# davidesantangelo/krep

Hardware: NVIDIA H100
Metric: GB/s scanned (HBM-resident corpus) (higher is better)
Workload: dtype u8

## Files before the change

krep_b200/csrc/engine.cu:

```cuda
#include <cub/device/device_radix_sort.cuh>
#include <algorithm>
#include <chrono>
#include <cstdarg>
#include <cstdio>
#include <cstdlib>
#include <cstring>
#include <mutex>
#include <thread>
#include "common.h"
#include "corpus.h"
#include "engine.h"

namespace kb {

static thread_local int t_err = 0;
static thread_local char t_errmsg[512] = "";

void set_error(int code, const char *fmt, ...)
{
    t_err = code;
    va_list ap;
    va_start(ap, fmt);
    vsnprintf(t_errmsg, sizeof t_errmsg, fmt, ap);
    va_end(ap);
// ... 128 lines not shown
    if (e != cudaSuccess)
    {
        cudaGetLastError();
        n = 0;
    }
    trace("cudaGetDeviceCount -> %d", n);
    g_visible = n > MAX_DEV ? MAX_DEV : n;
    return g_visible;
}

int primary_device()
{
    if (g_primary >= 0) return g_primary;
    if (visible_devices() == 0)
    {
        set_error(-1, "no CUDA device available; this engine has no CPU fallback");
        return -1;
    }
    int d = 0;
    if (cudaGetDevice(&d) != cudaSuccess) d = 0;
    g_primary = d;
    return d;
}

static int ctx_create(DevCtx &E, int device)
{
    trace("device %d: creating context", device);
    CK(cudaSetDevice(device));
    cudaDeviceProp prop;
    CK(cudaGetDeviceProperties(&prop, device));
    if (prop.major != 9 || prop.minor != 0)
    {
        set_error(-1, "device %d (%s, sm_%d%d) is not an sm_90 part; kernels are built for sm_90a only", device,
                  prop.name, prop.major, prop.minor);
        return -1;
    }
    E.device = device;
    E.sm_count = prop.multiProcessorCount;
    CK(cudaStreamCreateWithFlags(&E.scan_stream, cudaStreamNonBlocking));
    CK(cudaStreamCreateWithFlags(&E.copy_stream, cudaStreamNonBlocking));
    CK(cudaStreamCreateWithFlags(&E.fin_stream, cudaStreamNonBlocking));
    CK(cudaMalloc(&E.d_counter, 64 * SCAN_SLOTS));
    CK(cudaMemset(E.d_counter, 0, 64 * SCAN_SLOTS));
    CK(cudaEventCreate(&E.ev_ca));
    CK(cudaEventCreate(&E.ev_cb));
    for (int s = 0; s < SCAN_SLOTS; s++)
    {
        CK(cudaMalloc(&E.d_pack[s], (PACK_KEYS + 1) * sizeof(uint64_t)));
        CK(cudaHostAlloc(&E.h_pack[s], (PACK_KEYS + 1) * sizeof(uint64_t), cudaHostAllocMapped | cudaHostAllocPortable));
        E.h_pack[s][0] = 0;
        CK(cudaEventCreate(&E.ev_a[s]));
        CK(cudaEventCreate(&E.ev_b[s]));
        CK(cudaEventCreateWithFlags(&E.ev_done[s], cudaEventDisableTiming));
        CK(cudaEventCreateWithFlags(&E.ev_scanned[s], cudaEventDisableTiming));
        E.counter_clean[s] = true;
    }
    E.ready = true;
    trace("device %d: context ready (%s, %d SMs)", device, prop.name, E.sm_count);
    return 0;
}

DevCtx *ctx_get(int device)
{
    if (device < 0 || device >= MAX_DEV || device >= visible_devices())
    {
        set_error(-1, visible_devices() == 0 ? "no CUDA device available; this engine has no CPU fallback"
                                               : "CUDA device %d is not visible to this process",
                  device);
        return nullptr;
    }
    DevCtx &E = g_ctx[device];
    if (E.ready)
    {
        cudaSetDevice(device);
        return &E;
    }
    static std::mutex mu[MAX_DEV];
    std::lock_guard<std::mutex> lk(mu[device]);
    if (!E.ready && ctx_create(E, device) != 0) return nullptr;
    return &E;
}

DevCtx *ctx_primary()
{
    const int d = primary_device();
    return d < 0 ? nullptr : ctx_get(d);
}

static std::vector<Plan *> g_all_plans;
static std::mutex g_plans_mu;

static void ctx_destroy(DevCtx &E)
{
    if (!E.ready) return;
    cudaSetDevice(E.device);
    cudaDeviceSynchronize();
    for (int s = 0; s < SCAN_SLOTS; s++) cudaFree(E.d_list[s]);
    cudaFree(E.d_alt);
    cudaFree(E.d_sort_tmp);
    cudaFree(E.d_bounds);
    cudaFreeHost(E.h_bounds);
    cudaFreeHost(E.h_batch);
    cudaFree(E.d_rx_batch);
    cudaFree(E.d_counter);
    cudaFree(E.d_ring);
    cudaFree(E.d_line_recs);
    cudaFree(E.d_line_out);
    cudaFreeHost(E.h_line_out);
    cudaFreeHost(E.h_keys);
    regex_pack_free(E);
    for (int s = 0; s < SCAN_SLOTS; s++)
    {
        cudaFree(E.d_pack[s]);
        cudaFreeHost(E.h_pack[s]);
        cudaEventDestroy(E.ev_a[s]);
        cudaEventDestroy(E.ev_b[s]);
        cudaEventDestroy(E.ev_done[s]);
        cudaEventDestroy(E.ev_scanned[s]);
    }
    for (auto &s : E.stage) cudaFreeHost(s.buf);
    for (auto &s : E.stage)
        if (s.ev) cudaEventDestroy(s.ev);
    for (auto ev : E.ev_pool) cudaEventDestroy(ev);
    for (auto ev : E.ring_landed) cudaEventDestroy(ev);
    for (auto ev : E.ring_scanned) cudaEventDestroy(ev);
    cudaEventDestroy(E.ev_ca);
    cudaEventDestroy(E.ev_cb);
    cudaStreamDestroy(E.scan_stream);
    cudaStreamDestroy(E.copy_stream);
    cudaStreamDestroy(E.fin_stream);
    E = DevCtx();
}

void plan_cache_clear();

void engine_shutdown()
{
    std::lock_guard<std::recursive_mutex> lk(g_mu);
    DeviceGuard guard;
    plan_cache_clear();
    {
        std::lock_guard<std::mutex> lp(g_plans_mu);
        for (Plan *p : g_all_plans)
            for (int d = 0; d < MAX_DEV; d++)
            {
                PlanDev &pd = p->dev[d];
                if (!pd.ready) continue;
                cudaSetDevice(d);
                cudaFree(pd.d_pat_val);
                cudaFree(pd.d_pat_mask);
                if (pd.ac) ac_free_device(pd.ac);
                pd = PlanDev();
            }
    }
    for (int d = 0; d < MAX_DEV; d++) ctx_destroy(g_ctx[d]);
    g_primary = -1;
}

int ensure_keys(DevCtx &E, uint64_t cap)
{
    if (cap <= E.key_cap) return 0;
    uint64_t ncap = E.key_cap ? E.key_cap : (1ull << 20);
    while (ncap < cap) ncap *= 2;
    CK(cudaDeviceSynchronize());
    for (int s = 0; s < SCAN_SLOTS; s++)
    {
        cudaFree(E.d_list[s]);
        E.d_list[s] = nullptr;
    }
    cudaFree(E.d_alt);
// ... 350 lines not shown
int reset_counter(DevCtx &E, int slot, cudaStream_t stream)
{
    if (E.counter_clean[slot]) return 0;
    CK(cudaMemsetAsync(slot_counter(E, slot), 0, 64, stream));
    E.counter_clean[slot] = true;
    return 0;
}

static constexpr int FIN_THREADS = 512, FIN_SLICES = 16, FIN_KEYS = FIN_THREADS / FIN_SLICES, FIN_PIECE = 2048;

__global__ void __launch_bounds__(FIN_THREADS) k_finish(unsigned long long *counter, const uint64_t *__restrict__ keys, uint64_t cap,
                                                        uint64_t *d_pack, int want_sort)
{
    __shared__ uint64_t s_keys[FIN_PIECE];
    __shared__ unsigned long long s_cnt;
    if (threadIdx.x == 0) s_cnt = counter[0];
    __syncthreads();
    const unsigned long long cnt = s_cnt;
    if (blockIdx.x == 0 && threadIdx.x == 0) d_pack[0] = cnt;
    const bool sorting = want_sort && cnt != 0 && cnt <= PACK_KEYS && cnt <= cap;
    const uint32_t n = sorting ? (uint32_t)cnt : 0u;
    const uint32_t idx = blockIdx.x * FIN_KEYS + threadIdx.x / FIN_SLICES, slice = threadIdx.x % FIN_SLICES;
    if (blockIdx.x * FIN_KEYS < n)
    {
        const uint64_t mine = idx < n ? keys[idx] : ~0ull;
        uint32_t rank = 0;
        for (uint32_t base = 0; base < n; base += FIN_PIECE)
        {
            const uint32_t m = n - base < FIN_PIECE ? n - base : FIN_PIECE;
            for (uint32_t j = threadIdx.x; j < FIN_PIECE; j += FIN_THREADS) s_keys[j] = j < m ? keys[base + j] : ~0ull;
            __syncthreads();
            const uint32_t mr = (m + 63u) & ~63u;
#pragma unroll 8
            for (uint32_t j = slice; j < mr; j += FIN_SLICES) rank += s_keys[j] < mine ? 1u : 0u;
            __syncthreads();
        }
#pragma unroll
        for (int o = 1; o < FIN_SLICES; o <<= 1) rank += __shfl_xor_sync(0xffffffffu, rank, o);
        if (idx < n && slice == 0) d_pack[1 + rank] = mine;
    }
    __syncthreads();
    if (threadIdx.x == 0)
    {
        __threadfence();
        const unsigned long long done = atomicAdd(&counter[1], 1ULL);
        if (done == gridDim.x - 1)
        {
            counter[0] = 0;
            counter[1] = 0;
        }
    }
}

int finish_scan(DevCtx &E, int slot, int want_sort, cudaStream_t stream)
{
    k_finish<<<PACK_KEYS / FIN_KEYS, FIN_THREADS, 0, stream>>>(slot_counter(E, slot), E.d_list[slot], E.key_cap, E.d_pack[slot],
                                                                 (want_sort && E.d_list[slot]) ? 1 : 0);
    CK(cudaGetLastError());
    CK(cudaMemcpyAsync(E.h_pack[slot], E.d_pack[slot], (want_sort ? PACK_KEYS + 1 : 1) * sizeof(uint64_t), cudaMemcpyDeviceToHost, stream));
    CK(cudaEventRecord(E.ev_done[slot], stream));
    count_launch();
    E.counter_clean[slot] = true;
    return 0;
}

int sort_keys(DevCtx &E, int slot, uint64_t n, int end_bit, cudaStream_t stream, const uint64_t **sorted)
{
    *sorted = E.d_list[slot];
    if (n < 2) return 0;
    cub::DoubleBuffer<uint64_t> db(E.d_list[slot], E.d_alt);
    size_t need = 0;
    CK(cub::DeviceRadixSort::SortKeys(nullptr, need, db, (int64_t)n, 0, end_bit, stream));
    if (need > E.sort_tmp_bytes)
    {
        CK(cudaStreamSynchronize(stream));
        cudaFree(E.d_sort_tmp);
        E.d_sort_tmp = nullptr;
        E.sort_tmp_bytes = 0;
        CK(cudaMalloc(&E.d_sort_tmp, need));
        E.sort_tmp_bytes = need;
    }
    CK(cub::DeviceRadixSort::SortKeys(E.d_sort_tmp, need, db, (int64_t)n, 0, end_bit, stream));
    *sorted = db.Current();
    return 0;
}

static int bits_for(uint64_t v)
{
    int b = 1;
    while (b < 64 && (v >> b)) b++;
    return b;
}

int key_end_bit(const Plan *plan, uint64_t max_offset, bool regex_matches)
{
    const int shift = plan->is_ac ? AC_END_SHIFT : regex_matches ? REGEX_MATCH_SHIFT : LIT_TAG_BITS;
    int b = bits_for(max_offset) + shift;
    return b > 64 ? 64 : b;
}

__global__ void __launch_bounds__(256) k_line_bounds(const uint8_t *__restrict__ text, uint64_t avail, uint64_t go,
                                                     const uint64_t *__restrict__ keys, uint64_t n, int is_ac, int has_prev,
                                                     int has_next, uint64_t *__restrict__ out)
{
    const uint64_t i = ((uint64_t)blockIdx.x * blockDim.x + threadIdx.x) >> 5;
    const int lane = threadIdx.x & 31;
    if (i >= n) return;
    auto start_of = [&](uint64_t key) -> uint64_t {
        if (!is_ac) return (key >> LIT_TAG_BITS) - go;
        return (key >> AC_END_SHIFT) - (1024 - ((key >> AC_LEN_SHIFT) & 1023)) - go;
    };
    const uint64_t s = start_of(keys[i]);
    const uint64_t lb = (!is_ac && i > 0) ? start_of(keys[i - 1]) : 0;
// ... 34 lines not shown
            break;
        }
    }
    if (lane == 0)
    {
        out[2 * i] = ls;
        out[2 * i + 1] = le;
    }
}

static int line_bounds(DevCtx &E, const Plan *plan, const krep_b200_shard_t *sh, const uint64_t *d_sorted, uint64_t n,
                       cudaStream_t stream, const uint64_t **d_bounds)
{
    *d_bounds = nullptr;
    if (n == 0) return 0;
    if (2 * n > E.bounds_cap)
    {
        CK(cudaStreamSynchronize(stream));
        cudaFree(E.d_bounds);
        E.d_bounds = nullptr;
        E.bounds_cap = 0;
        const uint64_t cap = 2 * n + n / 4 + 1024;
        CK(cudaMalloc(&E.d_bounds, cap * sizeof(uint64_t)));
        E.bounds_cap = cap;
    }
    const uint64_t threads = n * 32;
    const int has_prev = sh->prev_byte >= 0 && sh->prev_byte != '\n';
    const int has_next = sh->next_byte >= 0 && sh->next_byte != '\n';
    k_line_bounds<<<(unsigned)((threads + 255) / 256), 256, 0, stream>>>((const uint8_t *)sh->d_text, sh->avail_len, sh->global_offset,
                                                                        d_sorted, n, plan->is_ac ? 1 : 0, has_prev, has_next, E.d_bounds);
    CK(cudaGetLastError());
    count_launch();
    *d_bounds = E.d_bounds;
    return 0;
}

int scan_begin(DevCtx &E, const Plan *plan, const krep_b200_shard_t *sh, int want_positions, cudaStream_t stream, int *slot_out)
{
    if (!stream) stream = E.scan_stream;
    if (want_positions && ensure_keys(E, 1) != 0) return -2;
    const int slot = E.next_slot;
    if (E.pend[slot].active)
    {
        set_error(-3, "krep_b200_scan_shard_begin: %d scans are already in flight on device %d", SCAN_SLOTS, E.device);
        return -3;
    }
    CK(cudaStreamWaitEvent(stream, E.ev_done[slot], 0));
    if (reset_counter(E, slot, stream) != 0) return -2;
    CK(cudaEventRecord(E.ev_a[slot], stream));
    int rc = launch_scan(E, plan, sh, want_positions, stream, slot);
    if (rc != 0) return rc;
    CK(cudaEventRecord(E.ev_b[slot], stream));
    CK(cudaGetLastError());
    if (finish_scan(E, slot, want_positions, stream) != 0) return -2;
    PendingScan &P = E.pend[slot];
    P.active = true;
    P.plan = plan;
    P.shard = *sh;
    P.want_positions = want_positions;
    P.stream = stream;
    E.next_slot = (slot + 1) % SCAN_SLOTS;
    *slot_out = slot;
    return 0;
}

int scan_end(DevCtx &E, int slot, ScanOut *out)
{
    PendingScan &P = E.pend[slot];
    if (slot < 0 || slot >= SCAN_SLOTS || !P.active)
    {
        set_error(-3, "krep_b200_scan_shard_end: no scan in flight in slot %d", slot);
        return -3;
    }
    P.active = false;
    const Plan *plan = P.plan;
    const krep_b200_shard_t *sh = &P.shard;
    cudaStream_t stream = P.stream;
    reset_kernel_ms();
    for (int attempt = 0; attempt < 3; attempt++)
    {
        CK(cudaEventSynchronize(E.ev_done[slot]));
        const uint64_t cnt = E.h_pack[slot][0];
        float ms = 0.f;
        cudaEventElapsedTime(&ms, E.ev_a[slot], E.ev_b[slot]);
        add_kernel_ms(ms);
        *out = ScanOut();
        out->count = cnt;
        out->device = E.device;
        out->serial = ++E.serial;
        E.result_stream = stream;
        if (!P.want_positions) return 0;
        if (cnt <= E.key_cap)
        {
            int rc = 0;
            out->stored = cnt;
            if (cnt <= PACK_KEYS)
            {
                out->d_keys = E.d_pack[slot] + 1;
                out->h_sorted = E.h_pack[slot] + 1;
            }
            else
                rc = sort_keys(E, slot, cnt, key_end_bit(plan, sh->global_offset + sh->avail_len), stream, &out->d_keys);
            if (rc == 0 && plan->count_lines) rc = line_bounds(E, plan, sh, out->d_keys, cnt, stream, &out->d_bounds);
            return rc;
        }
        out->overflow = 1;
        for (int s2 = 0; s2 < SCAN_SLOTS; s2++)
            if (s2 != slot && E.pend[s2].active)
            {
                set_error(-3, "krep_b200_scan_shard_end: the occurrence list overflowed while another scan is in flight; end each "
                              "scan before beginning the next until the list has grown");
                return -3;
            }
        if (ensure_keys(E, cnt + cnt / 8 + 1024) != 0) return -2;
        if (reset_counter(E, slot, stream) != 0) return -2;
        CK(cudaEventRecord(E.ev_a[slot], stream));
        int rc = launch_scan(E, plan, sh, 1, stream, slot);
        if (rc != 0) return rc;
        CK(cudaEventRecord(E.ev_b[slot], stream));
        if (finish_scan(E, slot, 1, stream) != 0) return -2;
    }
    set_error(-4, "occurrence list kept overflowing");
    return -4;
}

int scan_shard(DevCtx &E, const Plan *plan, const krep_b200_shard_t *sh, int want_positions, cudaStream_t stream, ScanOut *out)
{
    int slot = 0;
    int rc = scan_begin(E, plan, sh, want_positions, stream, &slot);
    if (rc != 0) return rc;
    return scan_end(E, slot, out);
}

int fetch_keys(DevCtx &E, const ScanOut &so, const uint64_t **h)
{
    *h = nullptr;
    if (so.stored == 0) return 0;
    if (so.h_sorted)
    {
        *h = so.h_sorted;
        return 0;
    }
    if (so.stored > E.h_keys_cap)
    {
        cudaFreeHost(E.h_keys);
        E.h_keys = nullptr;
        E.h_keys_cap = 0;
        uint64_t cap = so.stored + so.stored / 4;
        if (cap < (1u << 16)) cap = 1u << 16;
        CK(cudaMallocHost(&E.h_keys, cap * sizeof(uint64_t)));
        E.h_keys_cap = cap;
    }
    cudaStream_t s = E.result_stream ? E.result_stream : E.scan_stream;
    CK(cudaMemcpyAsync(E.h_keys, so.d_keys, so.stored * sizeof(uint64_t), cudaMemcpyDeviceToHost, s));
    CK(cudaStreamSynchronize(s));
    *h = E.h_keys;
    return 0;
}

uint64_t merge_key_lists(const uint64_t *const *lists, const uint64_t *counts, uint32_t n_lists, uint64_t *dst)
{
    uint64_t total = 0;
    std::vector<uint64_t> cut;
    for (uint32_t i = 0; i < n_lists; i++)
    {
        if (counts[i] == 0) continue;
        if (dst + total != lists[i]) memmove(dst + total, lists[i], counts[i] * sizeof(uint64_t));
        cut.push_back(total);
        total += counts[i];
    }
    for (size_t i = 1; i < cut.size(); i++)
        if (dst[cut[i] - 1] > dst[cut[i]]) std::inplace_merge(dst, dst + cut[i], dst + (i + 1 < cut.size() ? cut[i + 1] : total));
    return total;
// ... 384 lines not shown
```

krep_b200/csrc/engine.h:

```cpp
#pragma once
#include <mutex>
#include <vector>
#include "common.h"

namespace kb {

static constexpr uint32_t PACK_KEYS = 16384;
static constexpr int SCAN_SLOTS = 2;

struct StageSlot
{
    uint8_t *buf = nullptr;
    cudaEvent_t ev = nullptr;
    bool in_flight = false;
};

struct PendingScan
{
    bool active = false;
    const Plan *plan = nullptr;
    krep_b200_shard_t shard;
    int want_positions = 0;
    cudaStream_t stream = nullptr;
};

struct RegexPackBufs;

struct DevCtx
{
    bool ready = false;
    int device = 0, sm_count = 0;
    cudaStream_t scan_stream = nullptr, copy_stream = nullptr;
    cudaStream_t fin_stream = nullptr;
    unsigned long long *d_counter = nullptr;
    bool counter_clean[SCAN_SLOTS] = {false, false};
    uint64_t *d_list[SCAN_SLOTS] = {nullptr, nullptr};
    uint64_t *d_alt = nullptr;
    uint64_t key_cap = 0;
    void *d_sort_tmp = nullptr;
    size_t sort_tmp_bytes = 0;
    uint64_t *d_bounds = nullptr;
    uint64_t bounds_cap = 0;
    uint64_t *h_bounds = nullptr;
    uint64_t h_bounds_cap = 0;
    uint64_t *d_pack[SCAN_SLOTS] = {nullptr, nullptr}, *h_pack[SCAN_SLOTS] = {nullptr, nullptr};
    cudaEvent_t ev_a[SCAN_SLOTS] = {nullptr, nullptr}, ev_b[SCAN_SLOTS] = {nullptr, nullptr};
    cudaEvent_t ev_done[SCAN_SLOTS] = {nullptr, nullptr};
    cudaEvent_t ev_scanned[SCAN_SLOTS] = {nullptr, nullptr};
    cudaEvent_t ev_ca = nullptr, ev_cb = nullptr;
    PendingScan pend[SCAN_SLOTS];
    int next_slot = 0;
    uint64_t serial = 0;
    cudaStream_t result_stream = nullptr;
    void *d_line_recs = nullptr;
    uint64_t line_recs_cap = 0;
    uint64_t *d_line_out = nullptr, *h_line_out = nullptr;
    uint64_t line_out_cap = 0;
    uint8_t *d_ring = nullptr;
    size_t ring_slot_bytes = 0;
    int ring_slots = 0;
    std::vector<cudaEvent_t> ring_landed, ring_scanned;
    std::vector<StageSlot> stage;
    size_t stage_bytes = 0;
    std::vector<cudaEvent_t> ev_pool;
    uint64_t *h_keys = nullptr;
    uint64_t h_keys_cap = 0;
    uint8_t *h_batch = nullptr;
    uint64_t h_batch_cap = 0;
    uint8_t *d_rx_batch = nullptr;
    size_t rx_batch_cap = 0;
    RegexPackBufs *rx_pack = nullptr;
};

struct RegexPackStats
{
    float scan_ms = 0.f, pack_ms = 0.f;
    uint64_t packed_bytes = 0;
};
int regex_scan_keys(DevCtx &E, const Plan *plan, const krep_b200_shard_t *shard, int mode, const char *who, uint64_t *cnt,
                    const uint64_t **d_sorted, uint64_t *device_lines);
int regex_pack_row(DevCtx &E, const krep_b200_shard_t *sh, int mode, const uint64_t *d_keys, uint64_t nkeys,
                   uint64_t device_lines, const void **d_row, uint64_t *row_bytes, float *pack_ms);
uint8_t *regex_pack_host_buffer(DevCtx &E, uint64_t bytes);
void regex_pack_free(DevCtx &E);

struct ErrState
{
    int code = 0;
    char msg[512] = "";
};
void get_error(ErrState *e);
void adopt_error(const ErrState &e);

std::recursive_mutex &engine_mutex();
int primary_device();
int visible_devices();
DevCtx *ctx_get(int device);
DevCtx *ctx_primary();
void engine_shutdown();
void prewarm_host_path(DevCtx &C);
void keep_devices_visible();
void warm_join();
bool warm_running();

struct DeviceGuard
{
    int saved = -1;
    DeviceGuard() { if (cudaGetDevice(&saved) != cudaSuccess) { saved = -1; cudaGetLastError(); } }
    ~DeviceGuard() { if (saved >= 0) cudaSetDevice(saved); }
};

Plan *plan_build(const search_params_t *P, int algo, bool only_matching);
Plan *regex_plan_build(const search_params_t *P, std::string *why);
void plan_free(Plan *p);
const PlanDev *plan_on_device(const Plan *p, DevCtx &C);
int resolve_algo(const search_params_t *P, int algo);

unsigned long long *slot_counter(DevCtx &C, int slot);
int scan_begin(DevCtx &C, const Plan *plan, const krep_b200_shard_t *sh, int want_positions, cudaStream_t stream, int *slot);
int scan_end(DevCtx &C, int slot, ScanOut *out);
int scan_shard(DevCtx &C, const Plan *plan, const krep_b200_shard_t *sh, int want_positions, cudaStream_t stream, ScanOut *out);
int finish_scan(DevCtx &C, int slot, int want_sort, cudaStream_t stream);
int ensure_keys(DevCtx &C, uint64_t cap);
int reset_counter(DevCtx &C, int slot, cudaStream_t stream);
int sort_keys(DevCtx &C, int slot, uint64_t n, int end_bit, cudaStream_t stream, const uint64_t **sorted);
int key_end_bit(const Plan *plan, uint64_t max_offset, bool regex_matches = false);
int fetch_keys(DevCtx &C, const ScanOut &so, const uint64_t **h);
void add_kernel_ms(float ms);
void reset_kernel_ms();
float get_kernel_ms();
void set_kernel_ms(float ms);
void trace(const char *fmt, ...);

bool count_lines_eligible(const Plan *plan, const search_params_t *P, int algo);
int ensure_line_out(DevCtx &C, uint64_t n);
int launch_count_lines(DevCtx &C, const Plan *plan, const krep_b200_shard_t *sh, cudaStream_t stream, uint64_t index);
uint64_t combine_line_records(const uint64_t *recs, size_t n);

uint64_t merge_key_lists(const uint64_t *const *lists, const uint64_t *counts, uint32_t n_lists, uint64_t *dst);

}
```

krep_b200/csrc/scan_count.cu:

```cuda
#include <algorithm>
#include "engine.h"
#include "lit_filters.cuh"

namespace kb {

enum : uint32_t
{
    LR_HAS_HIT = 1,
    LR_FIRST_OPEN = 2,
    LR_LAST_PENDING = 4,
    LR_HAS_NL = 8
};

struct LineRec
{
    uint32_t lines, flags;
};

struct CountDev
{
    LitDevParams p;
    uint64_t own_end;
    uint32_t part_groups, n_parts;
    uint32_t exact;
    uint32_t tail;
    LineRec *recs;
};

struct PartState
{
    uint32_t lines = 0;
    bool has_hit = false, first_open = false, pending = false, seen_nl = false;
    uint64_t covered_to = 0;
};

__device__ __noinline__ unsigned verify_exact_call(const LitDevParams &p, long long cand) { return verify_exact(p, cand); }

__device__ __forceinline__ uint32_t nl_nibble(uint32_t w)
{
    const uint32_t x = w ^ 0x0A0A0A0Au;
    const uint32_t y = ~(((x & 0x7F7F7F7Fu) + 0x7F7F7F7Fu) | x | 0x7F7F7F7Fu);
    return ((y >> 7) * 0x10204080u) >> 28;
}
__device__ __forceinline__ uint32_t nl_mask16(const uint4 &v)
{
    return nl_nibble(v.x) | (nl_nibble(v.y) << 4) | (nl_nibble(v.z) << 8) | (nl_nibble(v.w) << 12);
}
__device__ __forceinline__ uint32_t range_mask16(uint64_t unit, uint64_t lo, uint64_t hi)
{
    uint32_t m = 0xFFFFu;
    if (unit < lo) m = lo - unit >= 16 ? 0u : (m & ~((1u << (uint32_t)(lo - unit)) - 1u));
    if (unit + 16 > hi) m = hi <= unit ? 0u : (m & ((1u << (uint32_t)(hi - unit)) - 1u));
    return m;
}

__device__ __noinline__ bool scan_for_newline(const LitDevParams &p, uint64_t lo, uint64_t hi)
{
    const uint32_t lane = threadIdx.x & 31;
    if (hi > p.avail_len) hi = p.avail_len;
    for (uint64_t base = lo & ~15ull; base < hi; base += 512)
    {
        const uint64_t unit = base + 16ull * lane;
        uint32_t nm = 0;
        if (unit < hi && unit + 16 > lo)
        {
            if (unit + 16 <= p.avail_len) nm = nl_mask16(__ldg(reinterpret_cast<const uint4 *>(p.text + unit)));
            else
                for (uint64_t q = unit; q < p.avail_len; q++) nm |= (p.text[q] == '\n' ? 1u : 0u) << (uint32_t)(q - unit);
            nm &= range_mask16(unit, lo, hi);
        }
        if (__any_sync(0xffffffffu, nm != 0)) return true;
    }
    return false;
}

__device__ __forceinline__ void settle(const LitDevParams &p, PartState &S, uint64_t upto)
{
    if (S.covered_to < upto && (S.pending || (!S.has_hit && !S.seen_nl)))
        if (scan_for_newline(p, S.covered_to, upto))
        {
            S.pending = false;
            S.seen_nl = true;
        }
}

__device__ __forceinline__ void account(PartState &S, uint32_t hm, uint32_t nm)
{
    const uint32_t lane = threadIdx.x & 31;
    const bool has_nl = nm != 0;
    const uint32_t fnl = has_nl ? (uint32_t)__ffs(nm) - 1 : 0, lnl = has_nl ? 31u - (uint32_t)__clz(nm) : 0;
    const bool f = has_nl && (hm & ((1u << fnl) - 1u)) != 0;
    const bool l = has_nl && ((hm >> lnl) >> 1) != 0;
    uint32_t inner = 0;
    if (__popc(nm) >= 2)
    {
        uint32_t prev = fnl, rest = nm & (nm - 1);
        while (rest)
        {
            const uint32_t nx = (uint32_t)__ffs(rest) - 1;
            if (hm & (((1u << nx) - 1u) & ~((2u << prev) - 1u))) inner++;
            prev = nx;
            rest &= rest - 1;
        }
    }
    const uint32_t A = __ballot_sync(0xffffffffu, has_nl), T = __ballot_sync(0xffffffffu, !has_nl && hm != 0);
    const uint32_t F = __ballot_sync(0xffffffffu, f), Lm = __ballot_sync(0xffffffffu, l);
    uint32_t innersum = 0;
    if (__ballot_sync(0xffffffffu, inner != 0)) innersum = __reduce_add_sync(0xffffffffu, inner);
    if (A == 0)
    {
        if (T)
        {
            if (!S.pending)
            {
                S.lines++;
                if (!S.has_hit && !S.seen_nl) S.first_open = true;
            }
            S.pending = true;
            S.has_hit = true;
        }
        return;
    }
    const uint32_t j1 = (uint32_t)__ffs(A) - 1, jr = 31u - (uint32_t)__clz(A);
    if ((T & ((1u << j1) - 1u)) || ((F >> j1) & 1u))
    {
        if (!S.pending)
        {
            S.lines++;
            if (!S.has_hit && !S.seen_nl) S.first_open = true;
        }
        S.has_hit = true;
    }
    S.pending = false;
    S.seen_nl = true;
    bool gap = false;
    if (has_nl && lane != j1)
    {
        const uint32_t below = A & ((1u << lane) - 1u);
        const uint32_t pj = 31u - (uint32_t)__clz(below);
        const uint32_t between = ((1u << lane) - 1u) & ~((2u << pj) - 1u);
        gap = ((Lm >> pj) & 1u) || (T & between) || f;
    }
    const uint32_t G = __ballot_sync(0xffffffffu, gap);
    S.lines += (uint32_t)__popc(G) + innersum;
    if (G || innersum) S.has_hit = true;
    if (((Lm >> jr) & 1u) || ((T >> jr) >> 1))
    {
        S.lines++;
        S.has_hit = true;
        S.pending = true;
    }
}

__device__ __forceinline__ uint64_t pack_state(const PartState &S)
{
    return (uint64_t)S.lines | ((uint64_t)((S.has_hit ? 1u : 0u) | (S.first_open ? 2u : 0u) | (S.pending ? 4u : 0u) | (S.seen_nl ? 8u : 0u)) << 32);
}
__device__ __forceinline__ void unpack_state(uint64_t k, PartState &S)
{
    S.lines = (uint32_t)k;
    const uint32_t f = (uint32_t)(k >> 32);
    S.has_hit = f & 1u;
    S.first_open = f & 2u;
    S.pending = f & 4u;
    S.seen_nl = f & 8u;
}
__device__ __noinline__ uint64_t account_call(uint64_t packed, uint32_t hm, uint32_t nm)
{
    PartState S;
    unpack_state(packed, S);
    account(S, hm, nm);
    return pack_state(S);
}

template <bool WINDOW>
__device__ __noinline__ uint32_t hit_mask16(const CountDev &D, uint64_t unit, const uint4 &v, uint32_t nx)
{
    const LitDevParams &p = D.p;
    const uint32_t w[5] = {v.x, v.y, v.z, v.w, nx};
    uint32_t hm = 0;
    if (WINDOW)
    {
        const uint32_t mask = p.fold & p.win_mask, k0 = p.K[0];
#pragma unroll
        for (int k = 0; k < 4; k++)
#pragma unroll
            for (int r = 0; r < 4; r++)
            {
                const uint32_t win = r == 0 ? w[k] : __funnelshift_r(w[k], w[k + 1], 8 * r);
                if ((win & mask) == k0)
                {
                    const uint64_t st = unit + 4 * k + r;
                    const bool ok = D.exact ? (st >= p.own_begin && st < p.own_end && st + p.m <= p.avail_len)
                                            : verify_exact_call(p, (long long)st) != 0;
                    if (ok) hm |= 1u << (4 * k + r);
                }
            }
    }
    else
    {
#pragma unroll
        for (int k = 0; k < 4; k++)
#pragma unroll
            for (int d = 0; d < 4; d++)
                if ((w[k] & p.fold) == p.K[d] && verify_exact_call(p, (long long)(unit + 4 * k) - d)) hm |= 1u << (4 * k);
    }
    return hm;
}

__device__ __noinline__ PartState count_tail(const CountDev &D, PartState S, uint64_t cov, uint64_t nl_lo, uint64_t nl_hi, bool window)
{
    const LitDevParams &p = D.p;
    const uint32_t lane = threadIdx.x & 31;
    if (p.avail_len < p.emit_len && cov >= nl_hi) return S;
    const uint64_t last_start = p.avail_len >= p.emit_len ? p.avail_len - p.emit_len : 0;
    uint64_t end = nl_hi > last_start + 1 ? nl_hi : last_start + 1;
    if (!window && end < cov + 1) end = cov + 1;
    for (uint64_t base = cov; base < end; base += 32)
    {
        settle(p, S, base > nl_lo ? base : nl_lo);
        const uint64_t q = base + lane;
        uint32_t hm = 0, nm = 0;
        if (q < end)
        {
            if (p.avail_len >= p.emit_len && q >= p.tail_start && q <= last_start && verify_exact(p, (long long)q)) hm = 1;
            if (!window && q == cov && p.avail_len >= p.emit_len)
                for (uint64_t s = p.tail_start; s < cov && s <= last_start; s++)
                    if (verify_exact(p, (long long)s)) hm = 1;
            if (q >= nl_lo && q < nl_hi && q < p.avail_len && p.text[q] == '\n') nm = 1;
            if (nm) hm = 0;
        }
        account(S, hm, nm);
        S.covered_to = base + 32;
    }
    return S;
}

#ifndef KREP_B200_COUNT_MINB
#define KREP_B200_COUNT_MINB 3
#endif
template <bool WINDOW, bool FOLD, bool MASKED>
__global__ void __launch_bounds__(256, KREP_B200_COUNT_MINB) k_count_lines(const __grid_constant__ CountDev D)
{
    const LitDevParams &p = D.p;
    const uint4 *__restrict__ t4 = reinterpret_cast<const uint4 *>(p.text);
    const uint32_t lane = threadIdx.x & 31;
    const uint32_t warp_global = (blockIdx.x * blockDim.x + threadIdx.x) >> 5, total_warps = (gridDim.x * blockDim.x) >> 5;
    const uint32_t k0 = p.K[0], k1 = p.K[1], k2 = p.K[2], k3 = p.K[3], fold = p.fold, mask = p.win_mask;
    const uint32_t c1 = p.mulc[0], c2 = p.mulc[1], c3 = p.mulc[2];
    for (uint32_t pi = warp_global; pi < D.n_parts; pi += total_warps)
    {
        const uint64_t ga = p.group_begin + (uint64_t)pi * D.part_groups;
        uint64_t gb = ga + D.part_groups;
        if (gb > p.group_end) gb = p.group_end;
        const bool last_part = pi + 1 == D.n_parts;
        const uint64_t nl_lo = ga * 16 > p.own_begin ? ga * 16 : p.own_begin;
        const uint64_t nl_hi = (last_part || gb * 16 > D.own_end) ? D.own_end : gb * 16;
        PartState S;
        S.covered_to = nl_lo;
        for (uint64_t g = ga; g < gb; g += 128)
        {
            uint4 v[4];
            uint32_t nx[4];
            bool ok[4];
#pragma unroll
            for (int u = 0; u < 4; u++)
            {
                const uint64_t gi = g + 32 * u + lane;
                ok[u] = gi < gb;
                v[u] = ok[u] ? ld_stream(t4 + gi) : make_uint4(0u, 0u, 0u, 0u);
                nx[u] = 0;
                if (WINDOW && ok[u] && (lane == 31 || gi + 1 >= gb)) nx[u] = __ldg(reinterpret_cast<const uint32_t *>(t4 + gi + 1));
            }
            uint32_t cand = 0;
#pragma unroll
            for (int u = 0; u < 4; u++)
            {
                bool h;
                if (WINDOW)
                {
                    const uint32_t nb = __shfl_down_sync(0xffffffffu, v[u].x, 1);
                    if (!(lane == 31 || g + 32 * u + lane + 1 >= gb)) nx[u] = nb;
                    h = hit_vec_w<FOLD, MASKED>(v[u], nx[u], fold, mask, k0, c1, c2, c3);
                }
                else
                    h = hit_vec<FOLD>(v[u], fold, k0, k1, k2, k3);
                cand |= (h && ok[u]) ? (1u << u) : 0u;
            }
            const uint32_t any = __reduce_or_sync(0xffffffffu, cand);
            if (any)
            {
                const uint64_t tile_lo = g * 16;
                settle(p, S, tile_lo > nl_lo ? tile_lo : nl_lo);
                const bool inside = tile_lo >= nl_lo && tile_lo + 2048 <= nl_hi;
                uint64_t st = pack_state(S);
#pragma unroll
                for (int u = 0; u < 4; u++)
                {
                    const uint64_t unit = tile_lo + 512ull * u + 16ull * lane;
                    uint32_t hm = 0, nm = 0;
                    if (ok[u])
                    {
                        if ((cand >> u) & 1u) hm = hit_mask16<WINDOW>(D, unit, v[u], nx[u]);
                        nm = nl_mask16(v[u]);
                        if (!inside) nm &= range_mask16(unit, nl_lo, nl_hi);
                    }
                    st = account_call(st, hm, nm);
                }
                unpack_state(st, S);
                S.covered_to = tile_lo + 2048;
            }
        }
        if (last_part && D.tail) S = count_tail(D, S, gb * 16, nl_lo, nl_hi, WINDOW);
        uint32_t flags = 0;
        if (S.has_hit)
        {
            if (S.pending && S.covered_to < nl_hi && scan_for_newline(p, S.covered_to, nl_hi)) S.pending = false;
            flags = LR_HAS_HIT | (S.first_open ? LR_FIRST_OPEN : 0u) | (S.pending ? LR_LAST_PENDING : 0u) | LR_HAS_NL;
        }
        else
        {
            const bool nl = S.seen_nl || (S.covered_to < nl_hi && scan_for_newline(p, S.covered_to, nl_hi));
            flags = nl ? LR_HAS_NL : 0u;
        }
        if (lane == 0) D.recs[pi] = LineRec{S.lines, flags};
    }
}

__host__ __device__ __forceinline__ void append_rec(uint64_t &lines, uint32_t &flags, uint64_t blines, uint32_t bflags)
{
    const bool ah = flags & LR_HAS_HIT, bh = bflags & LR_HAS_HIT;
    if (!bh)
    {
        if (ah && (bflags & LR_HAS_NL)) flags &= ~(uint32_t)LR_LAST_PENDING;
        flags |= bflags & LR_HAS_NL;
        return;
    }
    if (!ah)
    {
        const bool had_nl = flags & LR_HAS_NL;
        lines = blines;
        flags = bflags | LR_HAS_NL * had_nl;
        if (had_nl) flags &= ~(uint32_t)LR_FIRST_OPEN;
        return;
    }
    lines += blines;
    if ((flags & LR_LAST_PENDING) && (bflags & LR_FIRST_OPEN)) lines--;
    flags = LR_HAS_HIT | LR_HAS_NL | (flags & LR_FIRST_OPEN) | (bflags & LR_LAST_PENDING);
}

__global__ void __launch_bounds__(1024) k_count_finish(const LineRec *recs, uint32_t n, uint64_t *d_out, uint64_t *h_out)
{
    __shared__ uint64_t s_lines[1024];
    __shared__ uint32_t s_flags[1024];
    const uint32_t per = (n + blockDim.x - 1) / blockDim.x;
    const uint32_t a = threadIdx.x * per, b = a + per < n ? a + per : n;
    uint64_t lines = 0;
    uint32_t flags = 0;
    for (uint32_t i = a; i < b; i++) append_rec(lines, flags, recs[i].lines, recs[i].flags);
    s_lines[threadIdx.x] = lines;
    s_flags[threadIdx.x] = flags;
    __syncthreads();
    if (threadIdx.x == 0)
    {
        lines = 0;
        flags = 0;
        for (uint32_t t = 0; t < blockDim.x; t++) append_rec(lines, flags, s_lines[t], s_flags[t]);
        d_out[0] = lines;
        d_out[1] = flags;
        h_out[0] = lines;
        h_out[1] = flags;
    }
}

#define CKC(call)                                                                                  \
    do                                                                                             \
    {                                                                                              \
        cudaError_t e_ = (call);                                                                   \
// ... 37 lines not shown
        set_error(-3, "shard text pointer must be 16-byte aligned");
        return -3;
    }
    const PlanDev *pd = plan_on_device(plan, E);
    if (!pd) return -2;
    if (ensure_line_out(E, index + 1) != 0) return -2;
    CountDev D;
    memset(&D, 0, sizeof D);
    LitDevParams &p = D.p;
    const uint64_t own_end = sh->own_end < sh->avail_len ? sh->own_end : sh->avail_len;
    p.text = (const uint8_t *)sh->d_text;
    p.avail_len = sh->avail_len;
    p.own_begin = sh->own_begin;
    p.own_end = own_end;
    p.global_offset = sh->global_offset;
    p.prev_byte = sh->prev_byte;
    p.next_byte = sh->next_byte;
    uint64_t total_groups;
    const bool window = plan->filter == FILTER_WINDOW4;
    if (!window)
    {
        total_groups = sh->avail_len / 16;
        p.tail_start = total_groups ? total_groups * 16 - 3 : 0;
    }
    else
    {
        total_groups = sh->avail_len >= 20 ? (sh->avail_len - 20) / 16 + 1 : 0;
        p.tail_start = total_groups * 16;
    }
    p.group_begin = sh->own_begin / 16;
    p.group_end = (own_end + 2) / 16 + 1;
    D.tail = p.group_end > total_groups ? 1u : 0u;
    if (p.group_end > total_groups) p.group_end = total_groups;
    if (p.group_begin > p.group_end) p.group_begin = p.group_end;
    p.m = plan->m;
    p.emit_len = plan->emit_len;
    for (int d = 0; d < 4; d++) p.K[d] = plan->K[d];
    p.fold = plan->fold;
    p.win_mask = plan->win_mask;
    p.mulc[0] = 1u << 24;
    p.mulc[1] = 1u << 16;
    p.mulc[2] = 1u << 8;
    p.pat_val = pd->d_pat_val;
    p.pat_mask = pd->d_pat_mask;
    p.whole_word = plan->whole_word;
    D.own_end = own_end;
    {
        bool letters = true;
        for (unsigned char ch : plan->pattern) letters &= is_alpha_c(ch);
        D.exact = (window && plan->m <= 4 && plan->whole_word == 0 && (plan->case_sensitive || letters)) ? 1u : 0u;
    }
    const uint64_t groups = p.group_end - p.group_begin;
    const char *v = getenv("KREP_B200_COUNT_PART_KB");
    const uint32_t kb_ = v && atoi(v) > 0 ? (uint32_t)atoi(v) : 64;
    uint64_t part = std::max<uint32_t>(128, kb_ * 64 / 128 * 128);
    const uint64_t max_parts = 1u << 18;
    if ((groups + part - 1) / part > max_parts) part = ((groups + max_parts - 1) / max_parts + 127) / 128 * 128;
    D.part_groups = (uint32_t)part;
    D.n_parts = (uint32_t)std::max<uint64_t>((groups + part - 1) / part, 1);
    if (D.n_parts > E.line_recs_cap)
    {
        CKC(cudaStreamSynchronize(stream));
        cudaFree(E.d_line_recs);
        E.d_line_recs = nullptr;
        E.line_recs_cap = 0;
        const uint64_t cap = std::max<uint64_t>(D.n_parts, 1u << 16);
        CKC(cudaMalloc(&E.d_line_recs, cap * sizeof(LineRec)));
        E.line_recs_cap = cap;
    }
    D.recs = (LineRec *)E.d_line_recs;
    const bool folded = plan->fold != 0xFFFFFFFFu, masked = plan->win_mask != 0xFFFFFFFFu;
    const uint64_t want_blocks = ((uint64_t)D.n_parts + 7) / 8;
    const unsigned grid = (unsigned)std::min<uint64_t>(want_blocks, (uint64_t)E.sm_count * KREP_B200_COUNT_MINB);
    if (!window)
    {
        if (folded) k_count_lines<false, true, false><<<grid, 256, 0, stream>>>(D);
        else k_count_lines<false, false, false><<<grid, 256, 0, stream>>>(D);
    }
    else if (folded)
    {
        if (masked) k_count_lines<true, true, true><<<grid, 256, 0, stream>>>(D);
        else k_count_lines<true, true, false><<<grid, 256, 0, stream>>>(D);
    }
    else
    {
        if (masked) k_count_lines<true, false, true><<<grid, 256, 0, stream>>>(D);
        else k_count_lines<true, false, false><<<grid, 256, 0, stream>>>(D);
    }
    CKC(cudaGetLastError());
    k_count_finish<<<1, 1024, 0, stream>>>(D.recs, D.n_parts, E.d_line_out + 2 * index, E.h_line_out + 2 * index);
    CKC(cudaGetLastError());
    count_launch(2);
    return 0;
}

uint64_t combine_line_records(const uint64_t *recs, size_t n)
{
    uint64_t lines = 0;
    uint32_t flags = 0;
    for (size_t i = 0; i < n; i++) append_rec(lines, flags, recs[2 * i], (uint32_t)recs[2 * i + 1]);
    return lines;
}

}
```

Baseline: 3108.

## Rewrite line-count accounting with per-lane bit tricks and async readback stream

Replaces the warp-wide PartState accounting (many ballots, noinline calls, settle scans) with a per-lane LaneCount using a carry-propagation bit trick to count hit lines, deferring first-line/newline resolution to the end of each partition. The hit-mask construction is templated on fold/mask and made branch-free, with verification only on candidate bits. Separately, the pack readback copy is moved to a dedicated finish stream, and the default count partition size grows from 64 KB to 256 KB. It risks correctness subtleties in the new line-boundary logic and reduced parallelism from larger partitions.

```diff
diff --git a/krep_b200/csrc/engine.cu b/krep_b200/csrc/engine.cu
--- a/krep_b200/csrc/engine.cu
+++ b/krep_b200/csrc/engine.cu
@@ -204,6 +204,7 @@
         CK(cudaEventCreate(&E.ev_a[s]));
         CK(cudaEventCreate(&E.ev_b[s]));
         CK(cudaEventCreateWithFlags(&E.ev_done[s], cudaEventDisableTiming));
+        CK(cudaEventCreateWithFlags(&E.ev_fin[s], cudaEventDisableTiming));
         CK(cudaEventCreateWithFlags(&E.ev_scanned[s], cudaEventDisableTiming));
         E.counter_clean[s] = true;
     }
@@ -268,6 +269,7 @@
         cudaEventDestroy(E.ev_a[s]);
         cudaEventDestroy(E.ev_b[s]);
         cudaEventDestroy(E.ev_done[s]);
+        cudaEventDestroy(E.ev_fin[s]);
         cudaEventDestroy(E.ev_scanned[s]);
     }
     for (auto &s : E.stage) cudaFreeHost(s.buf);
@@ -724,13 +726,20 @@
     }
 }
 
-int finish_scan(DevCtx &E, int slot, int want_sort, cudaStream_t stream)
+int finish_scan(DevCtx &E, int slot, int want_sort, cudaStream_t stream, cudaStream_t readback)
 {
     k_finish<<<PACK_KEYS / FIN_KEYS, FIN_THREADS, 0, stream>>>(slot_counter(E, slot), E.d_list[slot], E.key_cap, E.d_pack[slot],
                                                                  (want_sort && E.d_list[slot]) ? 1 : 0);
     CK(cudaGetLastError());
-    CK(cudaMemcpyAsync(E.h_pack[slot], E.d_pack[slot], (want_sort ? PACK_KEYS + 1 : 1) * sizeof(uint64_t), cudaMemcpyDeviceToHost, stream));
-    CK(cudaEventRecord(E.ev_done[slot], stream));
+    cudaStream_t cs = stream;
+    if (readback)
+    {
+        CK(cudaEventRecord(E.ev_fin[slot], stream));
+        CK(cudaStreamWaitEvent(readback, E.ev_fin[slot], 0));
+        cs = readback;
+    }
+    CK(cudaMemcpyAsync(E.h_pack[slot], E.d_pack[slot], (want_sort ? PACK_KEYS + 1 : 1) * sizeof(uint64_t), cudaMemcpyDeviceToHost, cs));
+    CK(cudaEventRecord(E.ev_done[slot], cs));
     count_launch();
     E.counter_clean[slot] = true;
     return 0;
@@ -871,7 +880,7 @@
     if (rc != 0) return rc;
     CK(cudaEventRecord(E.ev_b[slot], stream));
     CK(cudaGetLastError());
-    if (finish_scan(E, slot, want_positions, stream) != 0) return -2;
+    if (finish_scan(E, slot, want_positions, stream, E.fin_stream) != 0) return -2;
     PendingScan &P = E.pend[slot];
     P.active = true;
     P.plan = plan;
@@ -937,7 +946,7 @@
         int rc = launch_scan(E, plan, sh, 1, stream, slot);
         if (rc != 0) return rc;
         CK(cudaEventRecord(E.ev_b[slot], stream));
-        if (finish_scan(E, slot, 1, stream) != 0) return -2;
+        if (finish_scan(E, slot, 1, stream, E.fin_stream) != 0) return -2;
     }
     set_error(-4, "occurrence list kept overflowing");
     return -4;
diff --git a/krep_b200/csrc/engine.h b/krep_b200/csrc/engine.h
--- a/krep_b200/csrc/engine.h
+++ b/krep_b200/csrc/engine.h
@@ -46,6 +46,7 @@
     uint64_t *d_pack[SCAN_SLOTS] = {nullptr, nullptr}, *h_pack[SCAN_SLOTS] = {nullptr, nullptr};
     cudaEvent_t ev_a[SCAN_SLOTS] = {nullptr, nullptr}, ev_b[SCAN_SLOTS] = {nullptr, nullptr};
     cudaEvent_t ev_done[SCAN_SLOTS] = {nullptr, nullptr};
+    cudaEvent_t ev_fin[SCAN_SLOTS] = {nullptr, nullptr};
     cudaEvent_t ev_scanned[SCAN_SLOTS] = {nullptr, nullptr};
     cudaEvent_t ev_ca = nullptr, ev_cb = nullptr;
     PendingScan pend[SCAN_SLOTS];
@@ -120,7 +121,7 @@
 int scan_begin(DevCtx &C, const Plan *plan, const krep_b200_shard_t *sh, int want_positions, cudaStream_t stream, int *slot);
 int scan_end(DevCtx &C, int slot, ScanOut *out);
 int scan_shard(DevCtx &C, const Plan *plan, const krep_b200_shard_t *sh, int want_positions, cudaStream_t stream, ScanOut *out);
-int finish_scan(DevCtx &C, int slot, int want_sort, cudaStream_t stream);
+int finish_scan(DevCtx &C, int slot, int want_sort, cudaStream_t stream, cudaStream_t readback = nullptr);
 int ensure_keys(DevCtx &C, uint64_t cap);
 int reset_counter(DevCtx &C, int slot, cudaStream_t stream);
 int sort_keys(DevCtx &C, int slot, uint64_t n, int end_bit, cudaStream_t stream, const uint64_t **sorted);
diff --git a/krep_b200/csrc/scan_count.cu b/krep_b200/csrc/scan_count.cu
--- a/krep_b200/csrc/scan_count.cu
+++ b/krep_b200/csrc/scan_count.cu
@@ -27,11 +27,11 @@
     LineRec *recs;
 };
 
-struct PartState
-{
-    uint32_t lines = 0;
-    bool has_hit = false, first_open = false, pending = false, seen_nl = false;
-    uint64_t covered_to = 0;
+constexpr uint32_t NO_HIT = 0xFFFFFFFFu;
+struct LaneCount
+{
+    uint32_t lines = 0, first = NO_HIT;
+    bool open = false;
 };
 
 __device__ __noinline__ unsigned verify_exact_call(const LitDevParams &p, long long cand) { return verify_exact(p, cand); }
@@ -53,6 +53,12 @@
     if (unit + 16 > hi) m = hi <= unit ? 0u : (m & ((1u << (uint32_t)(hi - unit)) - 1u));
     return m;
 }
+__device__ __forceinline__ uint32_t lanemask_lt()
+{
+    uint32_t m;
+    asm("mov.u32 %0, %%lanemask_lt;" : "=r"(m));
+    return m;
+}
 
 __device__ __noinline__ bool scan_for_newline(const LitDevParams &p, uint64_t lo, uint64_t hi)
 {
@@ -74,151 +80,78 @@
     return false;
 }
 
-__device__ __forceinline__ void settle(const LitDevParams &p, PartState &S, uint64_t upto)
-{
-    if (S.covered_to < upto && (S.pending || (!S.has_hit && !S.seen_nl)))
-        if (scan_for_newline(p, S.covered_to, upto))
-        {
-            S.pending = false;
-            S.seen_nl = true;
-        }
-}
-
-__device__ __forceinline__ void account(PartState &S, uint32_t hm, uint32_t nm)
-{
-    const uint32_t lane = threadIdx.x & 31;
-    const bool has_nl = nm != 0;
-    const uint32_t fnl = has_nl ? (uint32_t)__ffs(nm) - 1 : 0, lnl = has_nl ? 31u - (uint32_t)__clz(nm) : 0;
-    const bool f = has_nl && (hm & ((1u << fnl) - 1u)) != 0;
-    const bool l = has_nl && ((hm >> lnl) >> 1) != 0;
-    uint32_t inner = 0;
-    if (__popc(nm) >= 2)
-    {
-        uint32_t prev = fnl, rest = nm & (nm - 1);
-        while (rest)
-        {
-            const uint32_t nx = (uint32_t)__ffs(rest) - 1;
-            if (hm & (((1u << nx) - 1u) & ~((2u << prev) - 1u))) inner++;
-            prev = nx;
-            rest &= rest - 1;
-        }
-    }
-    const uint32_t A = __ballot_sync(0xffffffffu, has_nl), T = __ballot_sync(0xffffffffu, !has_nl && hm != 0);
-    const uint32_t F = __ballot_sync(0xffffffffu, f), Lm = __ballot_sync(0xffffffffu, l);
-    uint32_t innersum = 0;
-    if (__ballot_sync(0xffffffffu, inner != 0)) innersum = __reduce_add_sync(0xffffffffu, inner);
-    if (A == 0)
-    {
-        if (T)
-        {
-            if (!S.pending)
-            {
-                S.lines++;
-                if (!S.has_hit && !S.seen_nl) S.first_open = true;
-            }
-            S.pending = true;
-            S.has_hit = true;
-        }
-        return;
-    }
-    const uint32_t j1 = (uint32_t)__ffs(A) - 1, jr = 31u - (uint32_t)__clz(A);
-    if ((T & ((1u << j1) - 1u)) || ((F >> j1) & 1u))
-    {
-        if (!S.pending)
-        {
-            S.lines++;
-            if (!S.has_hit && !S.seen_nl) S.first_open = true;
-        }
-        S.has_hit = true;
-    }
-    S.pending = false;
-    S.seen_nl = true;
-    bool gap = false;
-    if (has_nl && lane != j1)
-    {
-        const uint32_t below = A & ((1u << lane) - 1u);
-        const uint32_t pj = 31u - (uint32_t)__clz(below);
-        const uint32_t between = ((1u << lane) - 1u) & ~((2u << pj) - 1u);
-        gap = ((Lm >> pj) & 1u) || (T & between) || f;
-    }
-    const uint32_t G = __ballot_sync(0xffffffffu, gap);
-    S.lines += (uint32_t)__popc(G) + innersum;
-    if (G || innersum) S.has_hit = true;
-    if (((Lm >> jr) & 1u) || ((T >> jr) >> 1))
-    {
-        S.lines++;
-        S.has_hit = true;
-        S.pending = true;
-    }
-}
-
-__device__ __forceinline__ uint64_t pack_state(const PartState &S)
-{
-    return (uint64_t)S.lines | ((uint64_t)((S.has_hit ? 1u : 0u) | (S.first_open ? 2u : 0u) | (S.pending ? 4u : 0u) | (S.seen_nl ? 8u : 0u)) << 32);
-}
-__device__ __forceinline__ void unpack_state(uint64_t k, PartState &S)
-{
-    S.lines = (uint32_t)k;
-    const uint32_t f = (uint32_t)(k >> 32);
-    S.has_hit = f & 1u;
-    S.first_open = f & 2u;
-    S.pending = f & 4u;
-    S.seen_nl = f & 8u;
-}
-__device__ __noinline__ uint64_t account_call(uint64_t packed, uint32_t hm, uint32_t nm)
-{
-    PartState S;
-    unpack_state(packed, S);
-    account(S, hm, nm);
-    return pack_state(S);
-}
-
-template <bool WINDOW>
-__device__ __noinline__ uint32_t hit_mask16(const CountDev &D, uint64_t unit, const uint4 &v, uint32_t nx)
+__device__ __forceinline__ void count_step(LaneCount &C, uint32_t hm, uint32_t nm, uint32_t lane_lt)
+{
+    const uint32_t ev = hm | nm;
+    const uint32_t Eb = __ballot_sync(0xffffffffu, ev != 0);
+    const uint32_t Hb = __ballot_sync(0xffffffffu, hm > nm);
+    const uint32_t below = Eb & lane_lt;
+    const uint32_t fresh = below ? (~Hb >> (31u - (uint32_t)__clz(below))) & 1u : (C.open ? 0u : 1u);
+    C.lines += (uint32_t)__popc(((~ev & 0xFFFFu) + ((nm << 1) | fresh)) & hm);
+    if (Eb) C.open = (Hb >> (31u - (uint32_t)__clz(Eb))) & 1u;
+}
+
+template <bool WINDOW, bool FOLD, bool MASKED>
+__device__ __forceinline__ uint32_t hit_mask16(const CountDev &D, uint64_t unit, const uint4 &v, uint32_t nx, bool edge)
 {
     const LitDevParams &p = D.p;
     const uint32_t w[5] = {v.x, v.y, v.z, v.w, nx};
-    uint32_t hm = 0;
+    uint32_t cm = 0, hm = 0;
     if (WINDOW)
     {
-        const uint32_t mask = p.fold & p.win_mask, k0 = p.K[0];
+        const uint32_t k0 = p.K[0], mul[4] = {0u, p.mulc[0], p.mulc[1], p.mulc[2]};
 #pragma unroll
         for (int k = 0; k < 4; k++)
+        {
+            const uint32_t lo = FOLD ? w[k] & p.fold : w[k], hi = FOLD ? w[k + 1] & p.fold : w[k + 1];
 #pragma unroll
             for (int r = 0; r < 4; r++)
             {
-                const uint32_t win = r == 0 ? w[k] : __funnelshift_r(w[k], w[k + 1], 8 * r);
-                if ((win & mask) == k0)
-                {
-                    const uint64_t st = unit + 4 * k + r;
-                    const bool ok = D.exact ? (st >= p.own_begin && st < p.own_end && st + p.m <= p.avail_len)
-                                            : verify_exact_call(p, (long long)st) != 0;
-                    if (ok) hm |= 1u << (4 * k + r);
-                }
+                uint32_t win = r == 0 ? lo : hi * mul[r] + __umulhi(lo, mul[r]);
+                if (MASKED) win &= p.win_mask;
+                cm |= (win == k0 ? 1u : 0u) << (4 * k + r);
             }
+        }
+        if (D.exact)
+        {
+            if (edge) cm &= range_mask16(unit, p.own_begin, p.own_end);
+            return cm;
+        }
+        for (uint32_t c = cm; c; c &= c - 1)
+        {
+            const uint32_t b = (uint32_t)__ffs(c) - 1;
+            if (verify_exact_call(p, (long long)(unit + b))) hm |= 1u << b;
+        }
     }
     else
     {
 #pragma unroll
         for (int k = 0; k < 4; k++)
-#pragma unroll
-            for (int d = 0; d < 4; d++)
-                if ((w[k] & p.fold) == p.K[d] && verify_exact_call(p, (long long)(unit + 4 * k) - d)) hm |= 1u << (4 * k);
+        {
+            const uint32_t x = FOLD ? w[k] & p.fold : w[k];
+#pragma unroll
+            for (int d = 0; d < 4; d++) cm |= (x == p.K[d] ? 1u : 0u) << (4 * k + d);
+        }
+        for (uint32_t c = cm; c; c &= c - 1)
+        {
+            const uint32_t b = (uint32_t)__ffs(c) - 1, k = b >> 2, d = b & 3u;
+            if (!((hm >> (4 * k)) & 1u) && verify_exact_call(p, (long long)(unit + 4 * k) - (long long)d)) hm |= 1u << (4 * k);
+        }
     }
     return hm;
 }
 
-__device__ __noinline__ PartState count_tail(const CountDev &D, PartState S, uint64_t cov, uint64_t nl_lo, uint64_t nl_hi, bool window)
+__device__ __forceinline__ void count_tail(const CountDev &D, LaneCount &C, uint64_t cov, uint64_t nl_lo, uint64_t nl_hi,
+                                           uint64_t part_lo, uint32_t lane_lt, bool window)
 {
     const LitDevParams &p = D.p;
     const uint32_t lane = threadIdx.x & 31;
-    if (p.avail_len < p.emit_len && cov >= nl_hi) return S;
+    if (p.avail_len < p.emit_len && cov >= nl_hi) return;
     const uint64_t last_start = p.avail_len >= p.emit_len ? p.avail_len - p.emit_len : 0;
     uint64_t end = nl_hi > last_start + 1 ? nl_hi : last_start + 1;
     if (!window && end < cov + 1) end = cov + 1;
     for (uint64_t base = cov; base < end; base += 32)
     {
-        settle(p, S, base > nl_lo ? base : nl_lo);
         const uint64_t q = base + lane;
         uint32_t hm = 0, nm = 0;
         if (q < end)
@@ -230,10 +163,9 @@
             if (q >= nl_lo && q < nl_hi && q < p.avail_len && p.text[q] == '\n') nm = 1;
             if (nm) hm = 0;
         }
-        account(S, hm, nm);
-        S.covered_to = base + 32;
-    }
-    return S;
+        if (hm && C.first == NO_HIT) C.first = (uint32_t)(q - part_lo);
+        count_step(C, hm, nm, lane_lt);
+    }
 }
 
 #ifndef KREP_B200_COUNT_MINB
@@ -244,7 +176,7 @@
 {
     const LitDevParams &p = D.p;
     const uint4 *__restrict__ t4 = reinterpret_cast<const uint4 *>(p.text);
-    const uint32_t lane = threadIdx.x & 31;
+    const uint32_t lane = threadIdx.x & 31, lane_lt = lanemask_lt();
     const uint32_t warp_global = (blockIdx.x * blockDim.x + threadIdx.x) >> 5, total_warps = (gridDim.x * blockDim.x) >> 5;
     const uint32_t k0 = p.K[0], k1 = p.K[1], k2 = p.K[2], k3 = p.K[3], fold = p.fold, mask = p.win_mask;
     const uint32_t c1 = p.mulc[0], c2 = p.mulc[1], c3 = p.mulc[2];
@@ -256,8 +188,7 @@
         const bool last_part = pi + 1 == D.n_parts;
         const uint64_t nl_lo = ga * 16 > p.own_begin ? ga * 16 : p.own_begin;
         const uint64_t nl_hi = (last_part || gb * 16 > D.own_end) ? D.own_end : gb * 16;
-        PartState S;
-        S.covered_to = nl_lo;
+        LaneCount C;
         for (uint64_t g = ga; g < gb; g += 128)
         {
             uint4 v[4];
@@ -287,43 +218,54 @@
                     h = hit_vec<FOLD>(v[u], fold, k0, k1, k2, k3);
                 cand |= (h && ok[u]) ? (1u << u) : 0u;
             }
-            const uint32_t any = __reduce_or_sync(0xffffffffu, cand);
-            if (any)
+            const uint64_t tile_lo = g * 16;
+            const bool edge = !(tile_lo >= nl_lo && tile_lo + 2048 <= nl_hi);
+            const uint32_t cand_w = __reduce_or_sync(0xffffffffu, cand);
+            if (cand_w)
             {
-                const uint64_t tile_lo = g * 16;
-                settle(p, S, tile_lo > nl_lo ? tile_lo : nl_lo);
-                const bool inside = tile_lo >= nl_lo && tile_lo + 2048 <= nl_hi;
-                uint64_t st = pack_state(S);
 #pragma unroll
                 for (int u = 0; u < 4; u++)
                 {
                     const uint64_t unit = tile_lo + 512ull * u + 16ull * lane;
+                    if (!((cand_w >> u) & 1u) && !C.open) continue;
                     uint32_t hm = 0, nm = 0;
                     if (ok[u])
                     {
-                        if ((cand >> u) & 1u) hm = hit_mask16<WINDOW>(D, unit, v[u], nx[u]);
                         nm = nl_mask16(v[u]);
-                        if (!inside) nm &= range_mask16(unit, nl_lo, nl_hi);
+                        if (edge) nm &= range_mask16(unit, nl_lo, nl_hi);
                     }
-                    st = account_call(st, hm, nm);
+                    if ((cand_w >> u) & 1u)
+                    {
+                        if ((cand >> u) & 1u) hm = hit_mask16<WINDOW, FOLD, MASKED>(D, unit, v[u], nx[u], edge);
+                        if (hm && C.first == NO_HIT) C.first = (uint32_t)(unit - ga * 16) + (uint32_t)__ffs(hm) - 1;
+                        count_step(C, hm, nm, lane_lt);
+                    }
+                    else if (__any_sync(0xffffffffu, nm != 0))
+                        C.open = false;
                 }
-                unpack_state(st, S);
-                S.covered_to = tile_lo + 2048;
             }
-        }
-        if (last_part && D.tail) S = count_tail(D, S, gb * 16, nl_lo, nl_hi, WINDOW);
-        uint32_t flags = 0;
-        if (S.has_hit)
-        {
-            if (S.pending && S.covered_to < nl_hi && scan_for_newline(p, S.covered_to, nl_hi)) S.pending = false;
-            flags = LR_HAS_HIT | (S.first_open ? LR_FIRST_OPEN : 0u) | (S.pending ? LR_LAST_PENDING : 0u) | LR_HAS_NL;
-        }
+            else if (C.open)
+            {
+                uint32_t nm = 0;
+#pragma unroll
+                for (int u = 0; u < 4; u++)
+                    if (ok[u])
+                    {
+                        const uint32_t m = nl_mask16(v[u]);
+                        nm |= edge ? m & range_mask16(tile_lo + 512ull * u + 16ull * lane, nl_lo, nl_hi) : m;
+                    }
+                if (__any_sync(0xffffffffu, nm != 0)) C.open = false;
+            }
+        }
+        if (last_part && D.tail) count_tail(D, C, gb * 16, nl_lo, nl_hi, ga * 16, lane_lt, WINDOW);
+        const uint32_t lines = __reduce_add_sync(0xffffffffu, C.lines), first = __reduce_min_sync(0xffffffffu, C.first);
+        uint32_t flags;
+        if (first != NO_HIT)
+            flags = LR_HAS_HIT | LR_HAS_NL | (C.open ? LR_LAST_PENDING : 0u) |
+                    (scan_for_newline(p, nl_lo, ga * 16 + first) ? 0u : LR_FIRST_OPEN);
         else
-        {
-            const bool nl = S.seen_nl || (S.covered_to < nl_hi && scan_for_newline(p, S.covered_to, nl_hi));
-            flags = nl ? LR_HAS_NL : 0u;
-        }
-        if (lane == 0) D.recs[pi] = LineRec{S.lines, flags};
+            flags = scan_for_newline(p, nl_lo, nl_hi) ? LR_HAS_NL : 0u;
+        if (lane == 0) D.recs[pi] = LineRec{lines, flags};
     }
 }
 
@@ -467,7 +409,7 @@
     }
     const uint64_t groups = p.group_end - p.group_begin;
     const char *v = getenv("KREP_B200_COUNT_PART_KB");
-    const uint32_t kb_ = v && atoi(v) > 0 ? (uint32_t)atoi(v) : 64;
+    const uint32_t kb_ = v && atoi(v) > 0 ? (uint32_t)atoi(v) : 256;
     uint64_t part = std::max<uint32_t>(128, kb_ * 64 / 128 * 128);
     const uint64_t max_parts = 1u << 18;
     if ((groups + part - 1) / part > max_parts) part = ((groups + max_parts - 1) / max_parts + 127) / 128 * 128;
```

Measured after the change: 3117, median of 6. Within noise of the previous version (+0.3%).
